# hahnyuan/PTQ4ViT

Hardware: AMD Instinct MI355X
Metric: calibration throughput (wrapped modules calibrated per second), ViT-B/224 W8A8, 32 calibration images (higher is better)
Workload: dtype int8

## Files before the change

ptq4vit_amd/csrc/p4v_api.hip:

```cpp
#include <hip/hip_runtime.h>

#include <algorithm>
#include <atomic>
#include <climits>
#include <cstdarg>
#include <cstdio>
#include <condition_variable>
#include <cstring>
#include <deque>
#include <functional>
#include <thread>
#include <mutex>
#include <string>
#include <unordered_map>
#include <type_traits>
#include <vector>

#include "../../include/ptq4vit_hip.h"
#include "../../include/ptq4vit_hip_debug.h"
#include "p4v_kernels.h"

using namespace p4v;

namespace {
// ... 41 lines not shown

struct Arena {
    char* base;
    size_t cap, off, peak;
    size_t top;
    bool dry;
    size_t gap;
    Arena(void* b, size_t c) : base((char*)b), cap(c & ~(size_t)255), off(0), peak(0), top(0), dry(b == nullptr),
                               gap(g_arena_gap.load(std::memory_order_relaxed)) {
        if (!dry) g_arena_ranges.clear();
    }
    template <typename T> T* get(size_t n) {
        off = (size_t)rup((long)off, 256);
        T* p = dry ? nullptr : (T*)(base + off);
        if (gap && !dry) arena_note(off, off + n * sizeof(T));
        off += n * sizeof(T) + gap;
        if (off + top > peak) peak = off + top;
        return p;
    }
    char* get_top(size_t bytes) {
        top += (size_t)rup((long)bytes, 256) + gap;
        if (off + top > peak) peak = off + top;
        if (dry || top > cap) return nullptr;
        if (gap) arena_note(cap - top, cap - top + bytes);
        return base + cap - top;
    }
    bool ok() const { return dry || off + top <= cap; }
};
struct ArenaMark {
    Arena& a;
    const size_t off;
    explicit ArenaMark(Arena& a_) : a(a_), off(a_.off) {}
    ~ArenaMark() { a.off = off; }
};

struct StatRec { hipEvent_t a, b; int kind; double macs, alg; int stage, gx, gz; double ms, bytes; };
thread_local double g_alg_bytes = 0;
thread_local double g_alg_macs_cand = 0;
thread_local double g_exec_frac = 1.0;
thread_local bool g_stat_on = false;
thread_local std::vector<StatRec> g_stat_recs;
thread_local std::vector<StatRec> g_stat_done;
thread_local bool g_b1_keep = false;
thread_local std::vector<float> g_b1_totals;
enum PruneStage { STAGE_FULL = 0, STAGE_A = 1, STAGE_B1 = 2, STAGE_B2 = 3, STAGE_A2 = 4 };
thread_local int g_stage = STAGE_FULL;
thread_local p4v_kernel_stats g_stats = {};
thread_local long g_memo_hits = 0, g_memo_misses = 0;
std::atomic<long long> g_prune_cnt[4];
constexpr int VARIANT_KEPT = 1 | 2 | 4 | 2048 | 32768 | 65536 | 131072 | 524288 | 1048576 | 2097152 | 4194304 | 8388608 | 134217728;
std::atomic<int> g_variant_word{0};
#define g_variant (g_variant_word.load(std::memory_order_relaxed) & 0x3fffffff)
#define g_force_v1 ((g_variant_word.load(std::memory_order_relaxed) >> 30) & 1)
std::atomic<int> g_tune[16];
enum { TUNE_CG6 = 0, TUNE_CG2 = 1, TUNE_CG2G = 2, TUNE_CG7 = 3, TUNE_PRINT = 4, TUNE_ORDER7 = 5, TUNE_P6 = 6, TUNE_PLANE_GIB = 7, TUNE_EPI6W = 8,
       TUNE_LOOSE_PCT = 9, TUNE_SLICE_DIV = 10, TUNE_SLICE_SMALL = 11, TUNE_B1_PATH = 12, TUNE_TIER2 = 13, TUNE_TIER2_DIV = 14, TUNE_LOOSE_ROWS = 15 };
inline bool tune_b1_removed(int v) { return v == 1 || v == 2 || v == 3 || v == 5 || v == 6 || v == 8 || v == 10 || v == 12; }
inline int tune(int k) { return g_tune[k].load(std::memory_order_relaxed); }
inline bool b1_previous() { return tune(TUNE_B1_PATH) == 4; }

inline int ws_aligned(const void* p) {
    return ((uintptr_t)p % WS_ALIGN) == 0 ? 0 : fail(P4V_ERR_INVALID, "d_workspace must be aligned to %zu bytes", WS_ALIGN);
}

struct Group;
struct Ctx {
    hipStream_t st;
    Arena ws;
    bool dry;
    Group* grp = nullptr;
    int slot = 0;
    int par = 1;
    static Ctx on(void* stream, void* workspace, size_t bytes) { return Ctx{(hipStream_t)stream, Arena(workspace, bytes), false}; }
    static Ctx sizing() { return Ctx{nullptr, Arena(nullptr, 0), true}; }
    size_t sized_bytes() const { return ws.peak + 4096; }
};

struct StatInfo { int kind; double macs, alg; int stage, gx, gz; double bytes; };
struct QOp;
struct KernelDesc {
    hipError_t (*one)(const QOp&, hipStream_t);
    hipError_t (*many)(const QOp* const*, int, hipStream_t);
    int cap;
};
constexpr int QOP_PARAM_BYTES = 480;
struct QOp {
    enum Type : int { KERNEL, FILL, D2H, H2D, COPY2D, WAIT };
    int type = KERNEL;
    const KernelDesc* kd = nullptr;
    dim3 grid, block;
    unsigned lds = 0;
    alignas(16) char params[QOP_PARAM_BYTES];
    void* dst = nullptr; const void* src = nullptr; size_t bytes = 0; int value = 0;
    size_t dpitch = 0, spitch = 0, width = 0, height = 0;
    std::vector<char> payload;
    bool timed = false;
    bool heavy = false;
    StatInfo si{};
};
inline hipError_t lds_attr(const void* fn, unsigned lds, std::atomic<bool>& done) {
    if (lds <= 48 * 1024 || done.load(std::memory_order_acquire)) return hipSuccess;
    const hipError_t e = hipFuncSetAttribute(fn, hipFuncAttributeMaxDynamicSharedMemorySize, 160 * 1024);
    if (e == hipSuccess) done.store(true, std::memory_order_release);
    return e;
}
template <typename P, void (*K1)(P), void (*KG)(GroupArgs<P>)> struct Kern {
    static_assert(sizeof(P) <= QOP_PARAM_BYTES, "kernel parameter block larger than a queued operation holds");
    static hipError_t one(const QOp& op, hipStream_t st) {
        static std::atomic<bool> attr{false};
// ... 1116 lines not shown
    }
    if (ps.col.prepacked) {
        if (ps.col.expanded || pl.cin_fix != 0 || !ps.i8 || !ps.stores())
            return fail(P4V_ERR_INVALID, "prepacked column operand: the fixed row-major int8 plane of a forward pass only");
    } else if (!ps.col.expanded) CHK(pack_operand(c, ps, pl, b, ps.col, b.col, true, 0, 1));
    return 0;
}

int chunk_exec_frac(Ctx& c, const Pass& ps, const SweepPlan& pl, int c0, int nc) {
    g_exec_frac = 1.0;
    if (!(g_stat_on && ps.crange && !c.dry)) return 0;
    int h[2] = {0, 0};
    const bool host_knows = ps.host_hi > ps.host_lo;
    const bool one_cand = !host_knows && ps.host_len == 1;
    if (host_knows) { h[0] = ps.host_lo; h[1] = ps.host_hi; }
    else if (one_cand) { h[0] = c0; h[1] = c0 + 1; }
    else { CHK(q_d2h(c, h, ps.crange, sizeof h)); CHK(q_sync(c)); }
    const int lo = std::max(h[0], c0), hi = std::min(h[1], c0 + nc);
    g_exec_frac = (double)std::max(0, hi - lo) / (double)nc;
    const int* blk = pl.rblk ? pl.rblk : pl.rblk_z;
    if (blk && ps.nj <= 64 && !one_cand) {
        int hb[128];
        if (host_knows && ps.host_rblk && ps.nj <= MIR_BLK) std::copy(ps.host_rblk, ps.host_rblk + 2 * ps.nj, hb);
        else { CHK(q_d2h(c, hb, blk, sizeof(int) * 2 * ps.nj)); CHK(q_sync(c)); }
        double sum = 0;
        for (int j = 0; j < ps.nj; ++j) sum += std::max(0, std::min(std::min(hb[2 * j + 1], h[1]), c0 + nc) - std::max(std::max(hb[2 * j], h[0]), c0));
        g_exec_frac = sum / ((double)nc * ps.nj);
    }
    if (tune(TUNE_PRINT) > 0) fprintf(stderr, "[p4v] pruned stage: candidates [%d, %d) of %d  (M %d N %d K %d Z %d nj %d)\n", h[0], h[1], ps.eq_n, ps.Mrows, ps.Ncols, ps.K, ps.Z, ps.nj);
    return 0;
}

int sweep_chunk_stationary(Ctx& c, const Pass& ps, const SweepPlan& pl, const PassBufs& b, int c0, int nc) {
    const bool a_search = pl.a_search;
    const int Kp = pl.Kp;
    Sweep3Params q{};
    q.S = a_search ? b.col : b.row; q.s_zs = 0;
    q.T = a_search ? b.row : b.col; q.t_cs = 0; q.t_zs = 0;
    q.t_rs = (long)(pl.pairs ? ((nc + 1) & ~1) : nc) * Kp;
    q.ldk = Kp; q.ktiles = Kp / SW_BKB;
    q.S1 = b.S1; q.s_cs = ps.s_cs; q.sb_on_t = a_search ? 0 : 1; q.sb_div = std::max(1, ps.sb_div);
    q.bias = ps.bias ? ps.bias : b.zero_bias; q.bias_on_t = a_search ? 0 : 1;
    q.O = ps.O; q.Wt = ps.G ? ps.G : ps.O; q.wt_mode = ps.wt_mode;
    q.o_ss = a_search ? ps.o_ns : ps.o_ms; q.o_ts = a_search ? ps.o_ms : ps.o_ns;
    q.SR = a_search ? ps.Ncols : ps.Mrows; q.TR = a_search ? ps.Mrows : ps.Ncols;
    q.c0 = c0; q.c1 = c0 + nc; q.crange = ps.crange;
    q.part = b.part; q.p_cs = pl.p_cs; q.NG = pl.s3_groups;
    q.stiles = (a_search ? pl.Np : pl.Mp) / 128; q.ttiles = (a_search ? pl.Mp : pl.Np) / 128;
    q.dbg = g_variant & 3;
    if (pl.kind == SK_SWEEP5) {
        const int cgroups = choose_cgroups((long)q.stiles * q.ttiles, nc, q.ktiles, cu_slots(c, 256, SWEEP_RECORD_KIND[SK_SWEEP5]), 30.0, 0.15);
        return launch_sweep5(c, q, ps.epi, cgroups);
    }
    q.stiles = pl.s6_stiles; q.ttiles = pl.s6_ttiles; q.E = b.epi6; q.crange_blk = pl.rblk;
    const int epi6k = ps.cos6 ? (a_search ? EPI_COS : EPI_COS_T) : ps.epi;
    if (ps.cos6) q.NG = pl.cos6_Sp;
    const bool known = ps.crange && ps.host_hi > ps.host_lo;
    const int nc_known = known ? std::max(1, std::min(ps.host_hi, c0 + nc) - std::max(ps.host_lo, c0)) : nc;
    const double P6 = tune(TUNE_P6) > 0 ? 0.125 * tune(TUNE_P6) : 25.0;
    const int slots6 = cu_slots(c, 256, SWEEP_RECORD_KIND[SK_SWEEP6]);
    if (pl.rblk && known && ps.host_rblk && ps.nj <= 4) {
        const int tpb = ps.sb_div / 64;
        for (int j = 0; j < ps.nj;) {
            if (ps.host_rblk[2 * j + 1] <= ps.host_rblk[2 * j]) { ++j; continue; }
            int j1 = j, lo = INT_MAX, hi = 0;
            double fsum = 0;
            for (; j1 < ps.nj && ps.host_rblk[2 * j1 + 1] > ps.host_rblk[2 * j1]; ++j1) {
                const int l = std::max(ps.host_rblk[2 * j1], c0), h = std::min(ps.host_rblk[2 * j1 + 1], c0 + nc);
                lo = std::min(lo, l); hi = std::max(hi, h);
                fsum += std::max(0, h - l);
            }
            Sweep3Params qq = q;
            const int tt0 = j * tpb, tt1 = std::min(q.ttiles, j1 * tpb);
            qq.tile0 = tt0 * q.stiles; qq.ntile = (tt1 - tt0) * q.stiles;
            const int ncr = std::max(1, hi - lo);
            g_exec_frac = fsum / ((double)(j1 - j) * nc);
            int cg6 = choose_cgroups((long)qq.ntile, ncr, q.ktiles, slots6, P6, 0.14);
            if (tune(TUNE_CG6) > 0) cg6 = std::max(1, std::min(ncr, tune(TUNE_CG6)));
            if (tune(TUNE_PRINT) > 0) fprintf(stderr, "[p4v] sweep6 open blocks [%d, %d): tiles %d x %d ktiles %d cand %d -> cgroups %d\n", j, j1, q.stiles, tt1 - tt0, q.ktiles, ncr, cg6);
            if (hi > lo && qq.ntile > 0) CHK(launch_sweep6(c, qq, epi6k, cg6, ncr));
            j = j1;
        }
        return 0;
    }
    int cg6 = choose_cgroups((long)q.stiles * q.ttiles, nc_known, q.ktiles, slots6, P6, 0.14);
    if (tune(TUNE_CG6) > 0) cg6 = std::max(1, std::min(nc, tune(TUNE_CG6)));
    if (tune(TUNE_PRINT) > 0) fprintf(stderr, "[p4v] sweep6 tiles %d x %d ktiles %d cand %d (%d known) -> cgroups %d\n", q.stiles, q.ttiles, q.ktiles, nc, nc_known, cg6);
    return launch_sweep6(c, q, epi6k, cg6, known ? nc_known : 0);
}

int sweep_chunk_large_k(Ctx& c, const Pass& ps, const SweepPlan& pl, const PassBufs& b, int c0, int nc) {
    Sweep7Params q{};
    q.r_cs = ps.col.expanded ? pl.col_plane1 : 0;
    q.R = b.col - (long)c0 * q.r_cs;
    q.c_cs = ps.row.expanded ? pl.row_plane1 : 0;
    q.Cp = b.row - (long)c0 * q.c_cs;
    q.C2 = pl.kind == SK_SWEEP7_TWIN ? b.row2 : nullptr;
    q.ldk = pl.Kp; q.ktiles = pl.Kp / SW_BKB;
    q.S1 = b.S1; q.S2 = b.S2; q.s_cs = ps.s_cs; q.sb_div = ps.s_cs > 1 ? std::max(1, ps.sb_div) : (1 << 30);
    q.E = b.epi7;
    q.c0 = c0; q.c1 = c0 + nc; q.crange = ps.crange;
    q.part = b.part; q.p_cs = pl.p_cs; q.NG = ps.cos7 ? pl.cos6_Sp : pl.NpP;
    q.rtiles = pl.Np / 256; q.ctiles = pl.Mp / (ps.twin ? 128 : 256);
    int cg7 = choose_cgroups((long)q.rtiles * q.ctiles, nc, q.ktiles + 3, cu_slots(c, 256, SWEEP_RECORD_KIND[ps.twin ? SK_SWEEP7_TWIN : SK_SWEEP7]), 6.0, 0.62, 100);
    if (tune(TUNE_CG7) > 0) cg7 = std::max(1, std::min(nc, tune(TUNE_CG7)));
    q.order = tune(TUNE_ORDER7) > 0 ? tune(TUNE_ORDER7) - 1 : 1;
    if (tune(TUNE_PRINT) > 0) fprintf(stderr, "[p4v] sweep7 tiles %d x %d ktiles %d cand %d twin %d -> cgroups %d\n", q.rtiles, q.ctiles, q.ktiles, nc, (int)ps.twin, cg7);
// ... 2575 lines not shown
        if (r.kind == 1 || r.kind == 11) { g_stats.sweep_f32_ms += ms; g_stats.sweep_f32_launches++; g_stats.sweep_f32_macs += r.macs; g_stats.sweep_f32_alg_macs += r.alg; }
        hipEventDestroy(r.a);
        hipEventDestroy(r.b);
        r.ms = ms;
        g_stat_done.push_back(r);
    }
    g_stat_recs.clear();
    return 0;
}

int p4v_stats_reset(void) {
    int r = stats_drain();
    g_stats = p4v_kernel_stats{};
    g_stat_done.clear();
    g_memo_hits = 0; g_memo_misses = 0;
    return r;
}

int p4v_stats_get(p4v_kernel_stats* out) {
    if (!out) return fail(P4V_ERR_INVALID, "stats_get: null");
    int r = stats_drain();
    g_stats.memo_hits = g_memo_hits; g_stats.memo_misses = g_memo_misses;
    g_stats.event_overhead_ms = g_evt_overhead_ms;
    *out = g_stats;
    return r;
}

int p4v_stats_launches(p4v_launch_record* out, int64_t capacity, int64_t* count) {
    int r = stats_drain();
    if (r) return r;
    if (count) *count = (int64_t)g_stat_done.size();
    if (out)
        for (int64_t i = 0; i < capacity && i < (int64_t)g_stat_done.size(); ++i) {
            const StatRec& s = g_stat_done[(size_t)i];
            out[i] = p4v_launch_record{s.kind, s.stage, s.gx, s.gz, (double)s.ms, 2.0 * s.macs, 2.0 * s.alg, s.bytes};
        }
    return 0;
}

int p4v_prune_counters(int64_t* out4, int reset) {
    if (out4) for (int i = 0; i < 4; ++i) out4[i] = (int64_t)g_prune_cnt[i].load(std::memory_order_relaxed);
    if (reset) for (int i = 0; i < 4; ++i) g_prune_cnt[i].store(0, std::memory_order_relaxed);
    return 0;
}

int p4v_debug_set_variant(int variant, int force_generic) {
    if (variant < 0 || variant >= (1 << 30)) return fail(P4V_ERR_INVALID, "p4v_debug_set_variant: bad variant word");
    if (variant & ~VARIANT_KEPT) return fail(P4V_ERR_INVALID, "p4v_debug_set_variant: bits 0x%x select removed paths", variant & ~VARIANT_KEPT);
    g_variant_word.store(variant | (force_generic ? (1 << 30) : 0), std::memory_order_relaxed);
    return 0;
}

int p4v_debug_set_tuning(int key, int value) {
    if (key < 0 || key >= 16) return fail(P4V_ERR_INVALID, "p4v_debug_set_tuning: unknown key %d", key);
    if (key == TUNE_B1_PATH && tune_b1_removed(value)) return fail(P4V_ERR_INVALID, "p4v_debug_set_tuning: 12 = %d selects a removed path", value);
    g_tune[key].store(value, std::memory_order_relaxed);
    return 0;
}

int p4v_debug_set_arena_gap(size_t bytes) {
    if (bytes % 256) return fail(P4V_ERR_INVALID, "p4v_debug_set_arena_gap: %zu is not a multiple of the arena's 256-byte alignment", bytes);
    g_arena_gap.store(bytes, std::memory_order_relaxed);
    return 0;
}

int p4v_debug_arena_ranges(uint64_t* out, int cap) {
    const int n = (int)g_arena_ranges.size();
    for (int i = 0; out && i < std::min(n, cap); ++i) { out[2 * i] = g_arena_ranges[i].first; out[2 * i + 1] = g_arena_ranges[i].second; }
    return n;
}

static int planes_out(const FusedPlanes& m, uint64_t* out, const char* who, const char* call) {
    if (!out) return fail(P4V_ERR_INVALID, "%s: null pointer", who);
    out[0] = m.off1; out[1] = m.off2; out[2] = (uint64_t)m.rows; out[3] = (uint64_t)m.cols; out[4] = (uint64_t)m.twin;
    return m.rows > 0 ? 0 : fail(P4V_ERR_INVALID, "%s: no %s call on this thread yet", who, call);
}
int p4v_debug_mlp_planes(uint64_t* out) { return planes_out(g_mlp_planes, out, "p4v_debug_mlp_planes", "p4v_mlp_quant_forward"); }
int p4v_debug_attn_planes(uint64_t* out) { return planes_out(g_attn_planes, out, "p4v_debug_attn_planes", "p4v_attn_quant_forward / p4v_wattn_quant_forward"); }
int p4v_debug_qkv_planes(uint64_t* out) {
    const QkvPlanes& m = g_qkv_planes;
    if (!out) return fail(P4V_ERR_INVALID, "p4v_debug_qkv_planes: null pointer");
    const uint64_t v[9] = {m.off_q, m.off_k, m.off_v, (uint64_t)m.Z, (uint64_t)m.rows_q, (uint64_t)m.rows_k, (uint64_t)m.ld_qk, (uint64_t)m.rows_v, (uint64_t)m.ld_v};
    std::copy(v, v + 9, out);
    return m.Z > 0 ? 0 : fail(P4V_ERR_INVALID, "p4v_debug_qkv_planes: no p4v_qkv_attn_quant_forward call on this thread yet");
}

int p4v_debug_sos_sweep(const p4v_matmul_desc* desc, const float* d_A, const float* d_B, const float* d_out, const float* d_grad,
                        int n_cands, int c_lo, int c_hi, int known_cands, float* d_scores, void* d_workspace, size_t workspace_bytes,
                        void* stream) {
    if (!desc || !d_A || !d_B || !d_out || !d_scores || !d_workspace) return fail(P4V_ERR_INVALID, "p4v_debug_sos_sweep: null pointer");
    if (!desc->sos || n_cands < 1 || n_cands > 20 || !sos_split_ok(desc->M, desc->K, desc->N, false))
        return fail(P4V_ERR_INVALID, "p4v_debug_sos_sweep: a split-of-softmax matmul of the one-kernel split search, 1..20 candidates");
    const SosDebugSweep dbg{n_cands, c_lo, c_hi, known_cands, d_scores};
    float* d_split = nullptr;
    CHK(ws_aligned(d_workspace));
    HIPCHK(hipMalloc(&d_split, 2 * sizeof(float)));
    Ctx c = Ctx::on(stream, d_workspace, workspace_bytes);
    g_sos_debug = &dbg;
    const int rc = matmul_impl(desc, {.A = d_A, .B = d_B, .O = d_out, .G = d_grad, .A_iv = d_split + 1, .split = d_split}, Stage{ST_S1}, c);
    g_sos_debug = nullptr;
    (void)hipFree(d_split);
    return rc;
}

int p4v_debug_bound_totals(float* out, int64_t capacity, int64_t* count) {
    if (!out && !count) { g_b1_keep = true; g_b1_totals.clear(); return 0; }
    g_b1_keep = false;
// ... 141 lines not shown
```

ptq4vit_amd/csrc/p4v_kernels.h:

```cpp
#pragma once
#include <hip/hip_runtime.h>
#include <stdint.h>
#include <type_traits>

namespace p4v {

typedef int v4i __attribute__((ext_vector_type(4)));
typedef int v16i __attribute__((ext_vector_type(16)));
typedef float v4f __attribute__((ext_vector_type(4)));
typedef float v16f __attribute__((ext_vector_type(16)));
typedef float v2f __attribute__((ext_vector_type(2)));

#ifndef P4V_GROUP_KERNARG
#define P4V_GROUP_KERNARG (4096 - 256)
#endif
template <typename P> struct GroupArgs {
    static constexpr int CAP_RAW = (P4V_GROUP_KERNARG - 16) / (int)(sizeof(P) + 16);
    static constexpr int CAP = CAP_RAW > 64 ? 64 : CAP_RAW;
    int n;
    unsigned off[CAP + 1];
    unsigned gx[CAP], gy[CAP], gz[CAP];
    P p[CAP];
};
#define P4V_BIDX uint3{blockIdx.x, blockIdx.y, blockIdx.z}
// ... 1993 lines not shown
                        float da = uu - (float)acc[0][i][r] * s1a, db = uu - (float)acc[1][i][r] * s1b;
                        if (TWIN) { da -= (float)acc2[0][i][r] * s2a; db -= (float)acc2[1][i][r] * s2b; }
                        if (EPI == EPI_SQ_W) { const float ta = ww * da, tb = ww * db; suma = fmaf(ta, ta, suma); sumb = fmaf(tb, tb, sumb); }
                        else if (EPI == EPI_SQ) { suma = fmaf(da, da, suma); sumb = fmaf(db, db, sumb); }
                        else if (EPI == EPI_ABS) { suma += fabsf(da); sumb += fabsf(db); }
                        else { suma = fmaf(ww * da, da, suma); sumb = fmaf(ww * db, db, sumb); }
                        acc[0][i][r] = 0; acc[1][i][r] = 0;
                        if (TWIN) { acc2[0][i][r] = 0; acc2[1][i][r] = 0; }
                    }
                }
            suma = wave_sum_dpp(suma);
            sumb = wave_sum_dpp(sumb);
            if (lane == 63) { res[ci * 8 + wid] = suma; res[(ci + 1) * 8 + wid] = sumb; }
            kt = 0;
            ++pr;
        }
    };
    for (int it = 0; it < total; it += SW2_NS) {
        tile(it, std::integral_constant<int, 0>{});
        if (it + 1 < total) tile(it + 1, std::integral_constant<int, 1>{});
        if (it + 2 < total) tile(it + 2, std::integral_constant<int, 2>{});
        if (it + 3 < total) tile(it + 3, std::integral_constant<int, 3>{});
    }
    __syncthreads();
    for (int i = tid; i < ncand * 8; i += 512) {
        const int cc = c_lo + i / 8, wv = i % 8;
        p.part[(long)cc * p.p_cs + (long)z * p.p_zs + (long)(mt * 2 + (wv >> 2)) * p.Np + nt * 4 + (wv & 3)] = res[i];
    }
}
template <bool TWIN, int EPI>
__global__ __launch_bounds__(512, 2) void k_sweep2g(SweepParams p) { k_sweep2g_body<TWIN, EPI>(p, P4V_BIDX, P4V_GDIM); }
template <bool TWIN, int EPI>
__global__ __launch_bounds__(512, 2) void k_sweep2g_g(GroupArgs<SweepParams> a) { P4V_GROUP_ENTER(a); k_sweep2g_body<TWIN, EPI>(a.p[m_], vb_, vg_); }

struct Sweep3Params {
    const int* crange;
    const void* S; long s_zs;
    const void* T; long t_cs, t_zs;
    long t_rs;
    int ldk, ktiles;
    const float* S1;
    int s_cs, sb_on_t, sb_div;
    const float* bias; int bias_on_t;
    const float* O; const float* Wt; int wt_mode;
    long o_ss, o_ts;
    int SR, TR;
    int c0, c1;
    float* part; long p_cs; int NG;
    int stiles, ttiles;
    int dbg;
    int tile0, ntile;
    const float* E;
    const int* crange_blk;
#ifdef P4V_TRACE
    unsigned long long* trace;
#endif
};

static constexpr int SW5_NP = 3;

template <int EPI>
__device__ __forceinline__ void k_sweep5_body(const Sweep3Params& p, const uint3 blockIdx, const uint3 gridDim) {
    extern __shared__ __attribute__((aligned(16))) char smem[];
#ifdef P4V_TRACE
    unsigned long long* trc = p.trace + ((size_t)blockIdx.z * gridDim.x + blockIdx.x) * 16;
    if (threadIdx.x == 0) { trc[0] = __builtin_amdgcn_s_memrealtime(); trc[8] = __builtin_amdgcn_s_memtime(); trc[4] = __builtin_amdgcn_s_getreg((4 << 0) | (0 << 6) | (31 << 11)); trc[5] = __builtin_amdgcn_s_getreg((20 << 0) | (0 << 6) | (31 << 11)); }
#endif
    const int ktiles = p.ktiles;
    const int ring0 = ktiles * SW2_TILE;
    float* res = reinterpret_cast<float*>(smem + ring0 + SW5_NP * 2 * SW2_TILE);

    const int tid = threadIdx.x, lane = tid & 63;
    const int wid = __builtin_amdgcn_readfirstlane(tid >> 6);
    const int wr = wid >> 2, wc = wid & 3;
    const int g = lane >> 5, l31 = lane & 31;

    const int nwg = p.stiles * p.ttiles;
    const int t = xcd_remap(blockIdx.x, nwg);
    const int st = t % p.stiles, tt = t / p.stiles;
    const int s0 = st * 128, t0 = tt * 128;
    const CandSpan cspan = cand_span(p.c0, p.c1, p.crange, blockIdx.z, gridDim.z, true);
    const int c_lo = cspan.lo, c_hi = cspan.hi, per = cspan.per;
    if (c_lo >= c_hi) return;

    const int ld_row = wid * 16 + (lane >> 2);
    const int ld_chunk = (lane & 3) ^ ((ld_row >> 2) & 3);
    {
        const char* gS = (const char*)p.S + (long)(s0 + ld_row) * p.ldk + ld_chunk * 16;
        for (int kt = 0; kt < ktiles; ++kt) glds16(gS + kt * SW_BKB, smem + kt * SW2_TILE + wid * 1024);
    }
    const char* curT = (const char*)p.T + (long)(t0 + ld_row) * p.t_rs + (long)(c_lo - p.c0) * p.ldk + ld_chunk * 16;
    const int total = ((c_hi - c_lo + 1) >> 1) * ktiles;
#pragma unroll
    for (int i = 0; i < SW5_NP; ++i) {
        glds16(curT, smem + ring0 + i * 2 * SW2_TILE + wid * 1024);
        glds16(curT + SW_BKB, smem + ring0 + i * 2 * SW2_TILE + SW2_TILE + wid * 1024);
        curT += 2 * SW_BKB;
    }

    float u[2][16], w[2][16];
    {
        const int tr = t0 + wc * 32 + l31;
        const long toff = (long)min(tr, p.TR - 1) * p.o_ts;
#pragma unroll
        for (int i = 0; i < 2; ++i)
#pragma unroll
// ... 215 lines not shown
__global__ __launch_bounds__(256) void k_prep_epi6_g(GroupArgs<PrepEpi6Params> a) { P4V_GROUP_ENTER(a); k_prep_epi6_body(a.p[m_], vb_, vg_); }

#ifndef P4V_SW6_DBG
#define P4V_SW6_DBG 0
#endif
template <int EPI, int KT, int RB>
__device__ __forceinline__ void k_sweep6_body(const Sweep3Params& p, const uint3 blockIdx, const uint3 gridDim) {
    constexpr int NW = 8 / RB;
    constexpr bool COS = EPI == EPI_COS || EPI == EPI_COS_T, TR = EPI == EPI_COS_T;
    static_assert(RB == 2, "k_sweep6: one wave per SIMD (RB = 2) only");
    extern __shared__ __attribute__((aligned(16))) char smem[];
#ifdef P4V_TRACE
    unsigned long long* trc = p.trace + ((size_t)blockIdx.z * gridDim.x + blockIdx.x) * 16;
    if (threadIdx.x == 0) { trc[0] = __builtin_amdgcn_s_memrealtime(); trc[8] = __builtin_amdgcn_s_memtime(); trc[5] = __builtin_amdgcn_s_getreg((20 << 0) | (0 << 6) | (31 << 11)); }
#endif
    constexpr int KT_TILE = 64 * 64;
    constexpr int STG = KT * KT_TILE;
    float* res = reinterpret_cast<float*>(smem + 3 * STG);

    const int tid = threadIdx.x, lane = tid & 63;
    const int wid = __builtin_amdgcn_readfirstlane(tid >> 6);
    const int g = lane >> 5, l31 = lane & 31;

    const int nwg = p.ntile > 0 ? p.ntile : p.stiles * p.ttiles;
    const int t = p.tile0 + xcd_remap(blockIdx.x, nwg);
    const int st = t % p.stiles, tt = t / p.stiles;
    const int s0 = st * 256 + wid * (32 * RB), t0 = tt * 64;
    const CandSpan cspan = cand_span(p.c0, p.c1, p.crange, blockIdx.z, gridDim.z, p.crange_blk,
                                     [&] { return min((p.sb_on_t ? tt * 64 : st * 256) / p.sb_div, p.s_cs - 1); });
    const int c_lo = cspan.lo, c_hi = cspan.hi, per = cspan.per;
    if (c_lo >= c_hi) return;
    const int ncand = c_hi - c_lo;

    constexpr int NPC = 4 * KT;
    constexpr int PPW = (NPC + NW - 1) / NW;
    const int ld_row = (wid & 3) * 16 + (lane >> 2);
    const int ld_chunk = (lane & 3) ^ ((ld_row >> 2) & 3);
    const char* curT = (const char*)p.T + (long)(t0 + ld_row) * p.t_rs + (long)(c_lo - p.c0) * p.ldk + ld_chunk * 16;
    const int kt_w = wid >> 2;
    curT += kt_w * SW_BKB;
    auto piece = [&](const char* src, int stage_off, auto j_c) __attribute__((always_inline)) {
        constexpr int j = decltype(j_c)::value;
        constexpr int OFF = j * (NW / 4) * SW_BKB;
        const int kt = j * (NW / 4) + kt_w;
        if (NPC % NW == 0 || NW * j + wid < NPC)
            glds16_imm<OFF>(src, smem + stage_off + kt * KT_TILE + (wid & 3) * 1024 - OFF);
    };
    auto issue = [&](int stage_off) __attribute__((always_inline)) {
        [&]<int... J>(std::integer_sequence<int, J...>) __attribute__((always_inline)) {
            (piece(curT, stage_off, std::integral_constant<int, J>{}), ...);
        }(std::make_integer_sequence<int, PPW>{});
        curT += p.ldk;
    };
    issue(0);
    issue(STG);

    v4i sfr[KT][RB][2];
    {
        const v4i* gS = reinterpret_cast<const v4i*>(p.S) + (long)(s0 >> 6) * (KT * 4 * 64) + lane;
#pragma unroll
        for (int kt = 0; kt < KT; ++kt)
#pragma unroll
            for (int i = 0; i < RB; ++i)
#pragma unroll
                for (int h = 0; h < 2; ++h) {
                    if constexpr ((P4V_SW6_DBG & 32) != 0) sfr[kt][i][h] = v4i{lane, kt, i, h};
                    else sfr[kt][i][h] = gS[((kt * 2 + i) * 2 + h) * 64];
                }
        if constexpr (COS && KT * RB * 2 * 4 > 128) {
#pragma unroll
            for (int kt = 0; kt < KT; ++kt)
#pragma unroll
                for (int i = 0; i < RB; ++i)
#pragma unroll
                    for (int h = 0; h < 2; ++h) asm volatile("" : "+a"(sfr[kt][i][h]));
        }
    }

    float u[RB][2][16], w[RB][2][16];
    if constexpr (COS) {
        const v4f* gE = reinterpret_cast<const v4f*>(p.E) + ((long)t * 8 + wid * RB) * (2 * 4 * 2 * 64) + lane;
#pragma unroll
        for (int i = 0; i < RB; ++i)
#pragma unroll
            for (int cb = 0; cb < 2; ++cb)
#pragma unroll
                for (int q = 0; q < 4; ++q) {
                    const v4f u4 = gE[(((i * 2 + cb) * 4 + q) * 2 + 0) * 64];
#pragma unroll
                    for (int e = 0; e < 4; ++e) u[i][cb][q * 4 + e] = u4[e];
                    if ((TR && i == 0) || (!TR && cb == 0)) {
                        const v4f w4 = gE[(((i * 2 + cb) * 4 + q) * 2 + 1) * 64];
#pragma unroll
                        for (int e = 0; e < 4; ++e) w[i][cb][q * 4 + e] = w4[e];
                    }
                }
    } else if (p.E) {
        const v4f* gE = reinterpret_cast<const v4f*>(p.E) + ((long)t * 8 + wid * RB) * (2 * 4 * 2 * 64) + lane;
#pragma unroll
        for (int i = 0; i < RB; ++i)
#pragma unroll
            for (int cb = 0; cb < 2; ++cb)
#pragma unroll
                for (int q = 0; q < 4; ++q) {
                    v4f u4, w4;
                    if constexpr ((P4V_SW6_DBG & 16) != 0) { u4 = v4f{(float)lane, 1.f, 2.f, 3.f}; w4 = v4f{1.f, 1.f, 1.f, 1.f}; }
                    else {
                        u4 = gE[(((i * 2 + cb) * 4 + q) * 2 + 0) * 64];
                        w4 = gE[(((i * 2 + cb) * 4 + q) * 2 + 1) * 64];
                    }
#pragma unroll
                    for (int e = 0; e < 4; ++e) { u[i][cb][q * 4 + e] = u4[e]; w[i][cb][q * 4 + e] = w4[e]; }
                }
    } else {
        const unsigned m_g = p.wt_mode == 1 ? 0xffffffffu : 0u;
        const unsigned m_o = p.wt_mode == 2 ? 0xffffffffu : p.wt_mode == 3 ? 0x7fffffffu : 0u;
        const unsigned m_1 = p.wt_mode == 0 ? 0x3f800000u : 0u;
#pragma unroll
        for (int cb = 0; cb < 2; ++cb) {
            const int tr = t0 + cb * 32 + l31;
            const long toff = (long)min(tr, p.TR - 1) * p.o_ts;
            const float bias_t = p.bias[p.bias_on_t ? min(tr, p.TR - 1) : 0];
            const bool t_ok = tr < p.TR;
            float bs[RB][16];
#pragma unroll
            for (int i = 0; i < RB; ++i)
#pragma unroll
                for (int r = 0; r < 16; ++r) {
                    const int src = min(s0 + i * 32 + acc32_row(r, g), p.SR - 1);
                    const long idx = toff + (long)src * p.o_ss;
                    u[i][cb][r] = p.O[idx];
                    w[i][cb][r] = p.Wt[idx];
                    bs[i][r] = p.bias[p.bias_on_t ? 0 : src];
                }
#pragma unroll
            for (int i = 0; i < RB; ++i)
#pragma unroll
                for (int r = 0; r < 16; ++r) {
                    const bool ok = t_ok && (s0 + i * 32 + acc32_row(r, g)) < p.SR;
                    const float o = u[i][cb][r], gw = w[i][cb][r];
                    const float b = p.bias_on_t ? bias_t : bs[i][r];
                    const unsigned wbits = (__builtin_bit_cast(unsigned, gw) & m_g) | (__builtin_bit_cast(unsigned, o) & m_o) | m_1;
                    u[i][cb][r] = ok ? o - b : 0.0f;
                    w[i][cb][r] = ok ? __builtin_bit_cast(float, wbits) : 0.0f;
                }
        }
    }
    const int blk_row = p.sb_on_t ? t0 : s0;
    const int sb = __builtin_amdgcn_readfirstlane(min(blk_row / p.sb_div, p.s_cs - 1));
    float* s1tab = res + (per + 1) * (2 * NW);
    for (int i = lane; i < ncand; i += 64) s1tab[i * NW + wid] = p.S1 ? p.S1[(c_lo + i) * p.s_cs + sb] : 1.0f;

    float oo_fix[2] = {0.0f, 0.0f};
    auto half_sum = [](float x) __attribute__((always_inline)) {
        float y = x;
        asm volatile("s_nop 1\n\tv_permlane32_swap_b32 %0, %1" : "+v"(x), "+v"(y));
        return x + y;
    };
    if constexpr (COS) {
#pragma unroll
        for (int sg = 0; sg < 2; ++sg) {
            float t2 = 0.0f;
#pragma unroll
            for (int o = 0; o < 2; ++o)
#pragma unroll
                for (int r = 0; r < 16; ++r) { const float v = TR ? u[sg][o][r] : u[o][sg][r]; t2 = fmaf(v, v, t2); }
            oo_fix[sg] = half_sum(t2);
        }
    }
    float cd[2] = {0.0f, 0.0f}, cn[2] = {0.0f, 0.0f};
    float sd[2] = {0.0f, 0.0f}, sn[2] = {0.0f, 0.0f};
    const int Sp = p.NG;
    unsigned cos_row = 0;
    if constexpr (COS) cos_row = (unsigned)((TR ? tt * Sp + s0 + l31 : (st * 4 + wid) * Sp + t0 + l31) * 12);
    auto cos_store = [&](int cand, int sgrp, float d, float n2) __attribute__((always_inline)) {
        float* q = reinterpret_cast<float*>(reinterpret_cast<char*>(p.part + (long)cand * p.p_cs) + (cos_row + sgrp * 384));
        q[0] = d; q[1] = n2; q[2] = oo_fix[sgrp];
    };

    const int sw0 = (l31 >> 2) & 3;
    const unsigned lds0 = (unsigned)(unsigned long long)(__attribute__((address_space(3))) char*)smem;
    const unsigned tbase0 = lds0 + l31 * 64 + ((g ^ sw0) << 4);
    const unsigned tbase1 = lds0 + l31 * 64 + (((2 + g) ^ sw0) << 4);
    const unsigned s1addr0 = lds0 + 3 * STG + (per + 1) * (8 * NW) + wid * 4;
    float* dump = s1tab + per * NW;
    struct TF2 { v4i f[2]; };
    constexpr int PD = ((2 * KT) % 3 == 0) ? 2 : 3;
    constexpr int NB = PD + 1;
    TF2 tf[NB];
    static_assert((2 * KT) % NB == 0 && KT >= 3, "fragment ring needs 2 * KT divisible by the buffer count");
    constexpr int NSTEP = 2 * KT;
    constexpr int SBAR = (KT + KT / 2 < NSTEP - PD) ? KT + KT / 2 : NSTEP - PD;
    static_assert(SBAR >= KT && SBAR <= NSTEP - PD, "ring barrier must sit in phase 1, before the next candidate's first read");
    constexpr int NEL = RB * 16;
    constexpr int NSL = KT - 1;
    constexpr int EPS = (NEL + NSL - 1) / NSL;
    v16i acc[RB][2];
    const v16i zero16 = {0, 0, 0, 0, 0, 0, 0, 0, 0, 0, 0, 0, 0, 0, 0, 0};
#pragma unroll
    for (int i = 0; i < RB; ++i) acc[i][1] = zero16;
    float esum0 = 0.0f, esum1 = 0.0f;
    float ered = 0.0f, es1 = 1.0f, es1_next = 1.0f;
    auto epi_slice = [&](auto sl_c, auto cb_c, int slot) __attribute__((always_inline)) {
        constexpr int sl = decltype(sl_c)::value, cbE = decltype(cb_c)::value;
        if constexpr ((P4V_SW6_DBG & 4) != 0) {
// ... 5 lines not shown
        }
        if constexpr (COS) {
            if constexpr (sl == 0 && (!TR || cbE == 0)) { cd[0] = cd[1] = cn[0] = cn[1] = 0.0f; }
            if constexpr (sl < NSL) {
#pragma unroll
                for (int e = sl * EPS; e < (sl + 1) * EPS && e < NEL; ++e) {
                    const int i = e >> 4, r = e & 15;
                    const int sgi = TR ? i : 0;
                    const float o = fmaf((float)acc[i][cbE][r], es1, TR ? w[0][cbE][r] : w[i][0][r]);
                    cd[sgi] = fmaf(u[i][cbE][r], o, cd[sgi]);
                    cn[sgi] = fmaf(o, o, cn[sgi]);
                }
                if constexpr (TR) asm volatile("" : "+v"(cd[0]), "+v"(cd[1]), "+v"(cn[0]), "+v"(cn[1]));
                else asm volatile("" : "+v"(cd[0]), "+v"(cn[0]));
            } else if constexpr (!TR) {
                const float d = half_sum(cd[0]), n2 = half_sum(cn[0]);
                if constexpr (cbE == 1) { sd[0] = d; sn[0] = n2; }
                else {
                    cos_store(c_lo + slot - 1, 0, d, n2);
                    cos_store(c_lo + max(slot - 2, 0), 1, sd[0], sn[0]);
                }
            } else {
                if constexpr (cbE == 1) {
                    sd[0] = half_sum(cd[0]); sn[0] = half_sum(cn[0]); sd[1] = half_sum(cd[1]); sn[1] = half_sum(cn[1]);
                } else {
                    cos_store(c_lo + max(slot - 2, 0), 0, sd[0], sn[0]);
                    cos_store(c_lo + max(slot - 2, 0), 1, sd[1], sn[1]);
                }
            }
            return;
        }
        if constexpr (sl == 0) { esum0 = 0.0f; esum1 = 0.0f; }
        if constexpr (sl < NSL) {
#pragma unroll
            for (int e = sl * EPS; e < (sl + 1) * EPS && e < NEL; ++e) {
                const int i = e >> 4, r = e & 15;
                const float a = (float)acc[i][cbE][r];
                const float d = u[i][cbE][r] - a * es1;
                const float ww = w[i][cbE][r];
                float& es = (r & 1) ? esum1 : esum0;
                if (EPI == EPI_SQ_W) { const float t2 = ww * d; es = t2 * t2 + es; }
                else if (EPI == EPI_SQ) es = d * d + es;
                else if (EPI == EPI_ABS) es += fabsf(d);
                else es = (ww * d) * d + es;
            }
        } else {
            ered = wave_sum_dpp(esum0 + esum1);
            float* dst = (lane == 63) ? res + slot * (2 * NW) + wid * 2 + cbE : dump + lane;
            *dst = ered;
        }
    };
    const char* fillT = curT - p.ldk;
    int fill_stage = STG;
    auto step = [&](auto s_c, unsigned ad0, unsigned ad1, unsigned adn0, unsigned adn1, int ci) __attribute__((always_inline)) {
        constexpr int s = decltype(s_c)::value;
        constexpr int cb = s / KT, kt = s % KT;
        TF2& cur = tf[s % NB];
        TF2& pre = tf[(s + PD) % NB];
        constexpr int t = s + PD;
        if constexpr ((P4V_SW6_DBG & 8) != 0) {
        } else if constexpr (t < NSTEP) {
            P4V_DSR(pre.f[0], ad0, (t % KT) * KT_TILE + (t / KT) * 2048); P4V_DSR(pre.f[1], ad1, (t % KT) * KT_TILE + (t / KT) * 2048);
        } else {
            P4V_DSR(pre.f[0], adn0, (t - NSTEP) * KT_TILE); P4V_DSR(pre.f[1], adn1, (t - NSTEP) * KT_TILE);
        }
        if constexpr ((P4V_SW6_DBG & 8) != 0) {
            if constexpr (s == 0) { asm volatile("ds_read_b32 %0, %1" : "=v"(es1_next) : "v"(s1addr0 + ci * (4 * NW))); __builtin_amdgcn_s_waitcnt(0xC07F); }
        } else if constexpr (s == 0) {
            asm volatile("ds_read_b32 %0, %1" : "=v"(es1_next) : "v"(s1addr0 + ci * (4 * NW)));
            __builtin_amdgcn_s_waitcnt(0xC07F | ((2 * PD + 1) << 8));
        } else {
            __builtin_amdgcn_s_waitcnt(0xC07F | ((2 * PD) << 8));
        }
        asm volatile("" : "+v"(cur.f[0]), "+v"(cur.f[1]) :: "memory");
        if constexpr (s == KT) { asm volatile("" : "+v"(es1_next)); es1 = es1_next; }
#pragma unroll
        for (int h = 0; h < 2; ++h)
#pragma unroll
            for (int i = 0; i < RB; ++i) {
                if constexpr ((P4V_SW6_DBG & 2) == 0) {
                    if constexpr (TR) acc[i][cb] = __builtin_amdgcn_mfma_i32_32x32x32_i8(cur.f[h], sfr[kt][i][h], (kt == 0 && h == 0) ? zero16 : acc[i][cb], 0, 0, 0);
                    else acc[i][cb] = __builtin_amdgcn_mfma_i32_32x32x32_i8(sfr[kt][i][h], cur.f[h], (kt == 0 && h == 0) ? zero16 : acc[i][cb], 0, 0, 0);
                }
                if (h == 1 && i == 0) {
                    constexpr int P1 = NSTEP - SBAR;
                    constexpr int j = (s >= SBAR) ? s - SBAR : s + P1;
                    __builtin_amdgcn_sched_barrier(0x6);
                    if constexpr (j < PPW && (P4V_SW6_DBG & 1) == 0) piece(fillT, fill_stage, std::integral_constant<int, j>{});
                    __builtin_amdgcn_sched_barrier(0x6);
                }
            }
        if constexpr (cb == 0) epi_slice(std::integral_constant<int, kt>{}, std::integral_constant<int, 1>{}, ci);
        else epi_slice(std::integral_constant<int, kt>{}, std::integral_constant<int, 0>{}, ci + 1);
        __builtin_amdgcn_sched_barrier(0);
    };

    wait_vmcnt<0>();
    __builtin_amdgcn_s_barrier();
    int stage = 0;
    auto pro_read = [&](auto s_c) __attribute__((always_inline)) {
        constexpr int S = decltype(s_c)::value;
        TF2& d = tf[S];
        const unsigned b0 = tbase0, b1 = tbase1;
        P4V_DSR(d.f[0], b0, (S % KT) * KT_TILE + (S / KT) * 2048);
        P4V_DSR(d.f[1], b1, (S % KT) * KT_TILE + (S / KT) * 2048);
    };
    [&]<int... S>(std::integer_sequence<int, S...>) __attribute__((always_inline)) {
        (pro_read(std::integral_constant<int, S>{}), ...);
    }(std::make_integer_sequence<int, PD>{});
#ifdef P4V_TRACE
    if (threadIdx.x == 0) { trc[1] = __builtin_amdgcn_s_memrealtime(); trc[6] = trc[1]; }
#endif
    for (int ci = 0; ci < ncand; ++ci) {
        const int stage_n = (stage + STG == 3 * STG) ? 0 : stage + STG;
        const unsigned ad0 = tbase0 + stage, ad1 = tbase1 + stage, adn0 = tbase0 + stage_n, adn1 = tbase1 + stage_n;
        auto run = [&](auto lo_c, auto hi_c) __attribute__((always_inline)) {
            [&]<int... S>(std::integer_sequence<int, S...>) __attribute__((always_inline)) {
                (step(std::integral_constant<int, decltype(lo_c)::value + S>{}, ad0, ad1, adn0, adn1, ci), ...);
            }(std::make_integer_sequence<int, decltype(hi_c)::value - decltype(lo_c)::value>{});
        };
        constexpr int SB = SBAR;
        run(std::integral_constant<int, 0>{}, std::integral_constant<int, SB>{});
        wait_vmcnt<0>();
        __builtin_amdgcn_s_barrier();
        fill_stage = (stage_n + STG == 3 * STG) ? 0 : stage_n + STG;
        fillT = curT;
        curT += p.ldk;
        run(std::integral_constant<int, SB>{}, std::integral_constant<int, NSTEP>{});
        stage = stage_n;
    }
    [&]<int... S>(std::integer_sequence<int, S...>) __attribute__((always_inline)) {
        (epi_slice(std::integral_constant<int, S>{}, std::integral_constant<int, 1>{}, ncand), ...);
    }(std::make_integer_sequence<int, KT>{});
#ifdef P4V_TRACE
    if (threadIdx.x == 0) trc[2] = __builtin_amdgcn_s_memrealtime();
#endif
    if constexpr (COS) {
        if constexpr (!TR) cos_store(c_lo + ncand - 1, 1, sd[0], sn[0]);
        else { cos_store(c_lo + ncand - 1, 0, sd[0], sn[0]); cos_store(c_lo + ncand - 1, 1, sd[1], sn[1]); }
    }
    __syncthreads();
    if constexpr (COS) return;
    for (int i = tid; i < ncand * 8; i += 64 * NW) {
        const int ci = i / 8, wv = (i % 8) >> 1, cb = i & 1;
        const float* r = res + (ci + 1) * (2 * NW);
        p.part[(long)(c_lo + ci) * p.p_cs + (long)(st * 4 + wv) * p.NG + tt * 2 + cb] = r[wv * 2 + cb];
    }
#ifdef P4V_TRACE
    if (threadIdx.x == 0) { trc[3] = __builtin_amdgcn_s_memrealtime(); trc[7] = (unsigned long long)ncand; trc[9] = __builtin_amdgcn_s_memtime(); }
#endif
}
template <int EPI, int KT, int RB>
__global__ __launch_bounds__(256, 1) void k_sweep6(Sweep3Params p) { k_sweep6_body<EPI, KT, RB>(p, P4V_BIDX, P4V_GDIM); }
template <int EPI, int KT, int RB>
__global__ __launch_bounds__(256, 1) void k_sweep6_g(GroupArgs<Sweep3Params> a) { P4V_GROUP_ENTER(a); k_sweep6_body<EPI, KT, RB>(a.p[m_], vb_, vg_); }

struct Sweep7Params {
    const int* crange;
    const void* R;  long r_cs;
    const void* Cp; long c_cs;
    const void* C2;
    int ldk, ktiles;
    const float* S1; const float* S2;
    int s_cs, sb_div;
    const float* E;
    int c0, c1;
    float* part; long p_cs; int NG;
    int rtiles, ctiles, cgroups;
    int order;
    const float* twin_s;
};

#ifndef P4V_SW7_DBG
#define P4V_SW7_DBG 0
#endif
#ifndef P4V_SW7_FILL
#define P4V_SW7_FILL 4
#endif
static constexpr int SW7_NS = 4;
static constexpr int SW7_REGION = 256 * 64;
static constexpr int SW7_STAGE = 2 * SW7_REGION;

struct PrepEpiParams {
// ... 1860 lines not shown
```

Baseline: 687.3.

## Overlap sweep6 prologue loads with first candidate's MFMA steps

Sweep6's prologue no longer waits for all global loads before the first candidate. The S fragments go straight into AGPRs, and the epilogue image (u/w) loads are issued in pieces between the first candidate's MFMA steps. Fine-grained vmcnt waits gate each kt slice, and the first candidate is peeled into its own specialised path. The S1 table load also becomes per-lane global loads written to LDS via ds_write. An eager tuning knob restores the up-front image load. The cost is much more fragile hand-scheduled vmcnt counting, more registers, and a risk of miscounted waits.

```diff
diff --git a/ptq4vit_amd/csrc/p4v_api.hip b/ptq4vit_amd/csrc/p4v_api.hip
--- a/ptq4vit_amd/csrc/p4v_api.hip
+++ b/ptq4vit_amd/csrc/p4v_api.hip
@@ -117,9 +117,9 @@
 std::atomic<int> g_variant_word{0};
 #define g_variant (g_variant_word.load(std::memory_order_relaxed) & 0x3fffffff)
 #define g_force_v1 ((g_variant_word.load(std::memory_order_relaxed) >> 30) & 1)
-std::atomic<int> g_tune[16];
+std::atomic<int> g_tune[17];
 enum { TUNE_CG6 = 0, TUNE_CG2 = 1, TUNE_CG2G = 2, TUNE_CG7 = 3, TUNE_PRINT = 4, TUNE_ORDER7 = 5, TUNE_P6 = 6, TUNE_PLANE_GIB = 7, TUNE_EPI6W = 8,
-       TUNE_LOOSE_PCT = 9, TUNE_SLICE_DIV = 10, TUNE_SLICE_SMALL = 11, TUNE_B1_PATH = 12, TUNE_TIER2 = 13, TUNE_TIER2_DIV = 14, TUNE_LOOSE_ROWS = 15 };
+       TUNE_LOOSE_PCT = 9, TUNE_SLICE_DIV = 10, TUNE_SLICE_SMALL = 11, TUNE_B1_PATH = 12, TUNE_TIER2 = 13, TUNE_TIER2_DIV = 14, TUNE_LOOSE_ROWS = 15, TUNE_EAGER6 = 16 };
 inline bool tune_b1_removed(int v) { return v == 1 || v == 2 || v == 3 || v == 5 || v == 6 || v == 8 || v == 10 || v == 12; }
 inline int tune(int k) { return g_tune[k].load(std::memory_order_relaxed); }
 inline bool b1_previous() { return tune(TUNE_B1_PATH) == 4; }
@@ -1342,7 +1342,7 @@
         const int cgroups = choose_cgroups((long)q.stiles * q.ttiles, nc, q.ktiles, cu_slots(c, 256, SWEEP_RECORD_KIND[SK_SWEEP5]), 30.0, 0.15);
         return launch_sweep5(c, q, ps.epi, cgroups);
     }
-    q.stiles = pl.s6_stiles; q.ttiles = pl.s6_ttiles; q.E = b.epi6; q.crange_blk = pl.rblk;
+    q.stiles = pl.s6_stiles; q.ttiles = pl.s6_ttiles; q.E = b.epi6; q.crange_blk = pl.rblk; q.eager = tune(TUNE_EAGER6) > 0 ? 1 : 0;
     const int epi6k = ps.cos6 ? (a_search ? EPI_COS : EPI_COS_T) : ps.epi;
     if (ps.cos6) q.NG = pl.cos6_Sp;
     const bool known = ps.crange && ps.host_hi > ps.host_lo;
@@ -4024,7 +4024,7 @@
 }
 
 int p4v_debug_set_tuning(int key, int value) {
-    if (key < 0 || key >= 16) return fail(P4V_ERR_INVALID, "p4v_debug_set_tuning: unknown key %d", key);
+    if (key < 0 || key >= 17) return fail(P4V_ERR_INVALID, "p4v_debug_set_tuning: unknown key %d", key);
     if (key == TUNE_B1_PATH && tune_b1_removed(value)) return fail(P4V_ERR_INVALID, "p4v_debug_set_tuning: 12 = %d selects a removed path", value);
     g_tune[key].store(value, std::memory_order_relaxed);
     return 0;
diff --git a/ptq4vit_amd/csrc/p4v_kernels.h b/ptq4vit_amd/csrc/p4v_kernels.h
--- a/ptq4vit_amd/csrc/p4v_kernels.h
+++ b/ptq4vit_amd/csrc/p4v_kernels.h
@@ -2069,6 +2069,7 @@
     int tile0, ntile;
     const float* E;
     const int* crange_blk;
+    int eager;
 #ifdef P4V_TRACE
     unsigned long long* trace;
 #endif
@@ -2390,11 +2391,41 @@
         }(std::make_integer_sequence<int, PPW>{});
         curT += p.ldk;
     };
+    constexpr bool LAZY = !COS;
+    struct Pro {
+        static constexpr int img_upto(int s) { return s < 0 ? 0 : (71 - 5 * KT + 4 * s < 32 ? 71 - 5 * KT + 4 * s : 32); }
+        static constexpr int sfr_younger(int kt) { return 4 * (KT - 1 - kt) + KT + img_upto(kt - 1); }
+    };
+    static_assert(Pro::sfr_younger(0) == 5 * KT - 4 && Pro::sfr_younger(0) <= 63 && Pro::sfr_younger(1) <= 63 && Pro::sfr_younger(KT - 1) <= 63, "vmcnt has 6 bits");
+    static_assert(Pro::img_upto(0) > 0 && Pro::img_upto(KT - 1) == 32, "the whole image is issued in phase 0 of the first candidate");
+    const int blk_row = p.sb_on_t ? t0 : s0;
+    const int sb = __builtin_amdgcn_readfirstlane(min(blk_row / p.sb_div, p.s_cs - 1));
+    float* s1tab = res + (per + 1) * (2 * NW);
+    float s1r[2] = {1.0f, 1.0f};
+    if (p.S1) {
+#pragma unroll
+        for (int j = 0; j < 2; ++j) {
+            const float* a = p.S1 + (c_lo + min(lane + 64 * j, ncand - 1)) * p.s_cs + sb;
+            asm volatile("global_load_dword %0, %1, off" : "=v"(s1r[j]) : "v"(a) : "memory");
+        }
+    }
+    for (int i = lane + 128; i < ncand; i += 64) s1tab[i * NW + wid] = p.S1 ? p.S1[(c_lo + i) * p.s_cs + sb] : 1.0f;
     issue(0);
-    issue(STG);
 
     v4i sfr[KT][RB][2];
-    {
+    const unsigned v16 = (unsigned)lane * 16u;
+    if constexpr (LAZY) {
+        const char* sS = reinterpret_cast<const char*>(p.S) + (long)(s0 >> 6) * (KT * 4 * 1024);
+#pragma unroll
+        for (int kt = 0; kt < KT; ++kt)
+#pragma unroll
+            for (int i = 0; i < RB; ++i)
+#pragma unroll
+                for (int h = 0; h < 2; ++h) {
+                    if constexpr ((P4V_SW6_DBG & 32) != 0) sfr[kt][i][h] = v4i{lane, kt, i, h};
+                    else asm volatile("global_load_dwordx4 %0, %1, %2 offset:%3" : "=a"(sfr[kt][i][h]) : "v"(v16), "s"(sS + kt * 4096), "n"((i * 2 + h) * 1024) : "memory");
+                }
+    } else {
         const v4i* gS = reinterpret_cast<const v4i*>(p.S) + (long)(s0 >> 6) * (KT * 4 * 64) + lane;
 #pragma unroll
         for (int kt = 0; kt < KT; ++kt)
@@ -2414,8 +2445,35 @@
                     for (int h = 0; h < 2; ++h) asm volatile("" : "+a"(sfr[kt][i][h]));
         }
     }
+    issue(STG);
 
     float u[RB][2][16], w[RB][2][16];
+    v4f ue[2][RB][4], we[2][RB][4];
+    const char* sE = reinterpret_cast<const char*>(p.E) + ((long)t * 8 + wid * RB) * (2 * 4 * 2 * 1024);
+    auto img_load = [&](auto n_c) __attribute__((always_inline)) {
+        constexpr int n = decltype(n_c)::value, cb = n / 16, i = (n / 8) % 2, q = (n / 2) % 4, k = n % 2;
+        constexpr int chunk = ((i * 2 + cb) * 4 + q) * 2 + k;
+        v4f& d = k ? we[cb][i][q] : ue[cb][i][q];
+        const unsigned vo = v16;
+        const char* se = sE + (chunk & ~3) * 1024;
+        if constexpr ((P4V_SW6_DBG & 16) != 0) d = k ? v4f{1.f, 1.f, 1.f, 1.f} : v4f{(float)lane, 1.f, 2.f, 3.f};
+        else asm volatile("global_load_dwordx4 %0, %1, %2 offset:%3" : "=v"(d) : "v"(vo), "s"(se), "n"((chunk & 3) * 1024) : "memory");
+    };
+    auto img_issue = [&](auto lo_c, auto hi_c) __attribute__((always_inline)) {
+        [&]<int... N>(std::integer_sequence<int, N...>) __attribute__((always_inline)) {
+            (img_load(std::integral_constant<int, decltype(lo_c)::value + N>{}), ...);
+        }(std::make_integer_sequence<int, decltype(hi_c)::value - decltype(lo_c)::value>{});
+    };
+    auto img_land = [&](auto cb_c) __attribute__((always_inline)) {
+        constexpr int cb = decltype(cb_c)::value;
+#pragma unroll
+        for (int i = 0; i < RB; ++i) {
+            asm volatile("" : "+v"(ue[cb][i][0]), "+v"(ue[cb][i][1]), "+v"(ue[cb][i][2]), "+v"(ue[cb][i][3]),
+                              "+v"(we[cb][i][0]), "+v"(we[cb][i][1]), "+v"(we[cb][i][2]), "+v"(we[cb][i][3]));
+#pragma unroll
+            for (int r = 0; r < 16; ++r) { u[i][cb][r] = ue[cb][i][r >> 2][r & 3]; w[i][cb][r] = we[cb][i][r >> 2][r & 3]; }
+        }
+    };
     if constexpr (COS) {
         const v4f* gE = reinterpret_cast<const v4f*>(p.E) + ((long)t * 8 + wid * RB) * (2 * 4 * 2 * 64) + lane;
 #pragma unroll
@@ -2434,61 +2492,61 @@
                     }
                 }
     } else if (p.E) {
-        const v4f* gE = reinterpret_cast<const v4f*>(p.E) + ((long)t * 8 + wid * RB) * (2 * 4 * 2 * 64) + lane;
-#pragma unroll
-        for (int i = 0; i < RB; ++i)
-#pragma unroll
-            for (int cb = 0; cb < 2; ++cb)
-#pragma unroll
-                for (int q = 0; q < 4; ++q) {
-                    v4f u4, w4;
-                    if constexpr ((P4V_SW6_DBG & 16) != 0) { u4 = v4f{(float)lane, 1.f, 2.f, 3.f}; w4 = v4f{1.f, 1.f, 1.f, 1.f}; }
-                    else {
-                        u4 = gE[(((i * 2 + cb) * 4 + q) * 2 + 0) * 64];
-                        w4 = gE[(((i * 2 + cb) * 4 + q) * 2 + 1) * 64];
-                    }
-#pragma unroll
-                    for (int e = 0; e < 4; ++e) { u[i][cb][q * 4 + e] = u4[e]; w[i][cb][q * 4 + e] = w4[e]; }
-                }
     } else {
         const unsigned m_g = p.wt_mode == 1 ? 0xffffffffu : 0u;
         const unsigned m_o = p.wt_mode == 2 ? 0xffffffffu : p.wt_mode == 3 ? 0x7fffffffu : 0u;
         const unsigned m_1 = p.wt_mode == 0 ? 0x3f800000u : 0u;
+        float bs[RB][16], uo[2][RB][16], wo[2][RB][16], bias_t[2];
+        if (!p.bias_on_t) {
+#pragma unroll
+            for (int i = 0; i < RB; ++i)
+#pragma unroll
+                for (int r = 0; r < 16; ++r) bs[i][r] = p.bias[min(s0 + i * 32 + acc32_row(r, g), p.SR - 1)];
+        } else {
+#pragma unroll
+            for (int i = 0; i < RB; ++i)
+#pragma unroll
+                for (int r = 0; r < 16; ++r) bs[i][r] = 0.0f;
+        }
 #pragma unroll
         for (int cb = 0; cb < 2; ++cb) {
             const int tr = t0 + cb * 32 + l31;
             const long toff = (long)min(tr, p.TR - 1) * p.o_ts;
-            const float bias_t = p.bias[p.bias_on_t ? min(tr, p.TR - 1) : 0];
-            const bool t_ok = tr < p.TR;
-            float bs[RB][16];
+            bias_t[cb] = p.bias[p.bias_on_t ? min(tr, p.TR - 1) : 0];
 #pragma unroll
             for (int i = 0; i < RB; ++i)
 #pragma unroll
                 for (int r = 0; r < 16; ++r) {
                     const int src = min(s0 + i * 32 + acc32_row(r, g), p.SR - 1);
                     const long idx = toff + (long)src * p.o_ss;
-                    u[i][cb][r] = p.O[idx];
-                    w[i][cb][r] = p.Wt[idx];
-                    bs[i][r] = p.bias[p.bias_on_t ? 0 : src];
+                    uo[cb][i][r] = p.O[idx];
+                    wo[cb][i][r] = p.Wt[idx];
                 }
+        }
+#pragma unroll
+        for (int cb = 0; cb < 2; ++cb)
+#pragma unroll
+            for (int i = 0; i < RB; ++i)
+#pragma unroll
+                for (int r = 0; r < 16; r += 4)
+                    asm volatile("" : "+v"(uo[cb][i][r]), "+v"(uo[cb][i][r + 1]), "+v"(uo[cb][i][r + 2]), "+v"(uo[cb][i][r + 3]),
+                                      "+v"(wo[cb][i][r]), "+v"(wo[cb][i][r + 1]), "+v"(wo[cb][i][r + 2]), "+v"(wo[cb][i][r + 3]));
+#pragma unroll
+        for (int cb = 0; cb < 2; ++cb) {
+            const bool t_ok = t0 + cb * 32 + l31 < p.TR;
 #pragma unroll
             for (int i = 0; i < RB; ++i)
 #pragma unroll
                 for (int r = 0; r < 16; ++r) {
                     const bool ok = t_ok && (s0 + i * 32 + acc32_row(r, g)) < p.SR;
-                    const float o = u[i][cb][r], gw = w[i][cb][r];
-                    const float b = p.bias_on_t ? bias_t : bs[i][r];
+                    const float o = uo[cb][i][r], gw = wo[cb][i][r];
+                    const float b = p.bias_on_t ? bias_t[cb] : bs[i][r];
                     const unsigned wbits = (__builtin_bit_cast(unsigned, gw) & m_g) | (__builtin_bit_cast(unsigned, o) & m_o) | m_1;
-                    u[i][cb][r] = ok ? o - b : 0.0f;
-                    w[i][cb][r] = ok ? __builtin_bit_cast(float, wbits) : 0.0f;
+                    ue[cb][i][r >> 2][r & 3] = ok ? o - b : 0.0f;
+                    we[cb][i][r >> 2][r & 3] = ok ? __builtin_bit_cast(float, wbits) : 0.0f;
                 }
         }
     }
-    const int blk_row = p.sb_on_t ? t0 : s0;
-    const int sb = __builtin_amdgcn_readfirstlane(min(blk_row / p.sb_div, p.s_cs - 1));
-    float* s1tab = res + (per + 1) * (2 * NW);
-    for (int i = lane; i < ncand; i += 64) s1tab[i * NW + wid] = p.S1 ? p.S1[(c_lo + i) * p.s_cs + sb] : 1.0f;
-
     float oo_fix[2] = {0.0f, 0.0f};
     auto half_sum = [](float x) __attribute__((always_inline)) {
         float y = x;
@@ -2600,8 +2658,10 @@
     };
     const char* fillT = curT - p.ldk;
     int fill_stage = STG;
-    auto step = [&](auto s_c, unsigned ad0, unsigned ad1, unsigned adn0, unsigned adn1, int ci) __attribute__((always_inline)) {
+    const bool lazy = LAZY && p.E && !p.eager;
+    auto step = [&](auto s_c, auto first_c, unsigned ad0, unsigned ad1, unsigned adn0, unsigned adn1, int ci) __attribute__((always_inline)) {
         constexpr int s = decltype(s_c)::value;
+        constexpr bool FIRST = decltype(first_c)::value;
         constexpr int cb = s / KT, kt = s % KT;
         TF2& cur = tf[s % NB];
         TF2& pre = tf[(s + PD) % NB];
@@ -2622,6 +2682,9 @@
         }
         asm volatile("" : "+v"(cur.f[0]), "+v"(cur.f[1]) :: "memory");
         if constexpr (s == KT) { asm volatile("" : "+v"(es1_next)); es1 = es1_next; }
+        if constexpr (FIRST && s >= 1 && s < KT)
+            asm volatile("s_waitcnt vmcnt(%4)" : "+a"(sfr[kt][0][0]), "+a"(sfr[kt][0][1]), "+a"(sfr[kt][1][0]), "+a"(sfr[kt][1][1]) : "n"(Pro::sfr_younger(s)) : "memory");
+        if constexpr (FIRST && s == KT) { wait_vmcnt<16>(); img_land(std::integral_constant<int, 0>{}); }
 #pragma unroll
         for (int h = 0; h < 2; ++h)
 #pragma unroll
@@ -2634,16 +2697,27 @@
                     constexpr int P1 = NSTEP - SBAR;
                     constexpr int j = (s >= SBAR) ? s - SBAR : s + P1;
                     __builtin_amdgcn_sched_barrier(0x6);
-                    if constexpr (j < PPW && (P4V_SW6_DBG & 1) == 0) piece(fillT, fill_stage, std::integral_constant<int, j>{});
+                    if constexpr (FIRST && s < SBAR) {
+                        if constexpr (Pro::img_upto(s) > Pro::img_upto(s - 1)) {
+                            if (lazy) img_issue(std::integral_constant<int, Pro::img_upto(s - 1)>{}, std::integral_constant<int, Pro::img_upto(s)>{});
+                        }
+                    } else if constexpr (j < PPW && (P4V_SW6_DBG & 1) == 0) piece(fillT, fill_stage, std::integral_constant<int, j>{});
                     __builtin_amdgcn_sched_barrier(0x6);
                 }
             }
-        if constexpr (cb == 0) epi_slice(std::integral_constant<int, kt>{}, std::integral_constant<int, 1>{}, ci);
+        if constexpr (cb == 0) { if constexpr (!FIRST) epi_slice(std::integral_constant<int, kt>{}, std::integral_constant<int, 1>{}, ci); }
         else epi_slice(std::integral_constant<int, kt>{}, std::integral_constant<int, 0>{}, ci + 1);
         __builtin_amdgcn_sched_barrier(0);
     };
 
-    wait_vmcnt<0>();
+    if constexpr (LAZY) { if (p.E && p.eager) img_issue(std::integral_constant<int, 0>{}, std::integral_constant<int, 32>{}); }
+    if (!lazy) wait_vmcnt<0>();
+    if constexpr (LAZY)
+        asm volatile("s_waitcnt vmcnt(%4)" : "+a"(sfr[0][0][0]), "+a"(sfr[0][0][1]), "+a"(sfr[0][1][0]), "+a"(sfr[0][1][1]) : "n"(Pro::sfr_younger(0)) : "memory");
+    asm volatile("" : "+v"(s1r[0]), "+v"(s1r[1]));
+#pragma unroll
+    for (int j = 0; j < 2; ++j)
+        if (lane + 64 * j < ncand) asm volatile("ds_write_b32 %0, %1" :: "v"(s1addr0 + (lane + 64 * j) * (4 * NW)), "v"(s1r[j]) : "memory");
     __builtin_amdgcn_s_barrier();
     int stage = 0;
     auto pro_read = [&](auto s_c) __attribute__((always_inline)) {
@@ -2659,24 +2733,27 @@
 #ifdef P4V_TRACE
     if (threadIdx.x == 0) { trc[1] = __builtin_amdgcn_s_memrealtime(); trc[6] = trc[1]; }
 #endif
-    for (int ci = 0; ci < ncand; ++ci) {
+    auto candidate = [&](auto first_c, int ci) __attribute__((always_inline)) {
         const int stage_n = (stage + STG == 3 * STG) ? 0 : stage + STG;
         const unsigned ad0 = tbase0 + stage, ad1 = tbase1 + stage, adn0 = tbase0 + stage_n, adn1 = tbase1 + stage_n;
         auto run = [&](auto lo_c, auto hi_c) __attribute__((always_inline)) {
             [&]<int... S>(std::integer_sequence<int, S...>) __attribute__((always_inline)) {
-                (step(std::integral_constant<int, decltype(lo_c)::value + S>{}, ad0, ad1, adn0, adn1, ci), ...);
+                (step(std::integral_constant<int, decltype(lo_c)::value + S>{}, first_c, ad0, ad1, adn0, adn1, ci), ...);
             }(std::make_integer_sequence<int, decltype(hi_c)::value - decltype(lo_c)::value>{});
         };
         constexpr int SB = SBAR;
         run(std::integral_constant<int, 0>{}, std::integral_constant<int, SB>{});
         wait_vmcnt<0>();
+        if constexpr (decltype(first_c)::value) img_land(std::integral_constant<int, 1>{});
         __builtin_amdgcn_s_barrier();
         fill_stage = (stage_n + STG == 3 * STG) ? 0 : stage_n + STG;
         fillT = curT;
         curT += p.ldk;
         run(std::integral_constant<int, SB>{}, std::integral_constant<int, NSTEP>{});
         stage = stage_n;
-    }
+    };
+    if constexpr (LAZY) candidate(std::true_type{}, 0);
+    for (int ci = LAZY ? 1 : 0; ci < ncand; ++ci) candidate(std::false_type{}, ci);
     [&]<int... S>(std::integer_sequence<int, S...>) __attribute__((always_inline)) {
         (epi_slice(std::integral_constant<int, S>{}, std::integral_constant<int, 1>{}, ncand), ...);
     }(std::make_integer_sequence<int, KT>{});
```

After: 687.5 (median of 2 runs). About the same (+0.0%).
